# JARVIS-MoCap/JARVIS-HybridNet

Measured on AMD Instinct MI355X. Metric: multi-view frames/s (12cam 1280x1024, 23kpt, 64^3 grid), higher is better.
Workload: dtype f32; 1 GPU; BASELINE configs[2]: HybridNet 12-camera 1280x1024, 23 kpts, 64^3 grid, small/small; cameras=12, joints=23, grid=64, streams=3, parallelism=single GPU, 3 time batches in flight on 3 HIP streams, hipgraph=False

## Files before the change

include/jarvis_hip.h:

```cpp
#ifndef JARVIS_HIP_H
#define JARVIS_HIP_H
#include <stdint.h>

#ifdef __cplusplus
extern "C" {
#endif

#define JH_ABI_VERSION 4

const char* jh_last_error(void);
int jh_abi_version(void);

#define JH_PRECISION_DEFAULT (-1)
#define JH_PRECISION_F32 0
#define JH_PRECISION_BF16X3 1
#define JH_PRECISION_BF16X3_WIDE 2
int jh_set_precision(int mode);
int jh_get_precision(void);

typedef struct jh_params jh_params;
int jh_params_create(jh_params** out);
int jh_params_set(jh_params* p, const char* key, const float* host, int64_t numel);
void jh_params_destroy(jh_params* p);

// ... 222 lines not shown
  const float *se_wr_host, *se_br_host, *se_we_host, *se_be_host;
  const double* se_pool_host;
} jh_op_operand;
int jh_op_conv_operand(int nd, int kind, int k, int stride, int pad, int cin, int cout,
                       const float* w_host, const float* b_host, const float* x_dev, int n, int d, int h,
                       int w, const float* gate_dev, const jh_op_operand* operand, float* y_dev, void* stream);
int jh_op_se_gate(const double* pool_host, int n, int c, int squeeze, float inv_hw, const float* wr_host,
                  const float* br_host, const float* we_host, const float* be_host, float* gate_dev, void* stream);
int jh_op_norm_apply(const float* x_dev, int n, int c, int d, int h, int w, const double* sums_host, int act,
                     const float* r1_dev, const double* r1_sums_host, const float* r2_dev, int write_y, int want_pool,
                     int min_block_kb, float* y_dev, double* pool_host, void* stream);
int jh_op_depthwise(int k, int c, const float* w_host, const float* x_dev, int n, int h, int w,
                    int norm_act, float* y_dev, void* stream);
int jh_op_depthwise_pool(int k, int c, const float* w_host, const float* x_dev, int n, int h, int w,
                         float* y_dev, float* pool_dev, void* stream);

int jh_op_yuv420_to_bgr(const uint8_t* frames_dev, int format, int n, int h, int w, uint8_t* out_bgr_dev,
                        void* stream);
int jh_op_yuv_surface_to_bgr(const uint8_t* frames_dev, const jh_yuv_surface* surface, int n, int h, int w,
                             uint8_t* out_bgr_dev, void* stream);
int jh_op_sensor_to_bgr(const uint8_t* frames_dev, const jh_sensor_surface* surface, int n, int h, int w,
                        uint8_t* out_bgr_dev, void* stream);

int64_t jh_joint_argmax_all_workspace_bytes(int n, int hh, int wh, int jp);
int jh_op_joint_argmax_all(const float* heat_dev, int n, int hh, int wh, int j, int jp, int32_t* idx_dev,
                           float* max_dev, void* workspace_dev, int64_t workspace_bytes, void* stream);

int jh_op_bifpn_node(int n_in, const int* modes, const float* weights, int act, int n, int c, int cout,
                     int h, int w, const float* x0_dev, const float* x1_dev, const float* x2_dev,
                     const float* dw_host, const float* pw_host, const float* bias_host, float* y_dev,
// ... 7 lines not shown
```

jarvis-hybridnet_amd/_native.py:

```python
import ctypes
import math
import os
from typing import NamedTuple

import torch

_HERE = os.path.dirname(os.path.abspath(__file__))
LIB_PATH = os.environ.get("JH_LIBRARY_PATH") or os.path.join(_HERE, "libjarvis_hip.so")
_lib = None

c_void_p, c_int, c_float, c_int64 = ctypes.c_void_p, ctypes.c_int, ctypes.c_float, ctypes.c_int64
c_char_p = ctypes.c_char_p


class PredictorConfig(ctypes.Structure):
    _fields_ = [("num_cameras", ctypes.c_int32), ("num_joints", ctypes.c_int32),
                ("center_size", ctypes.c_int32), ("bbox", ctypes.c_int32),
                ("roi_cube_size", c_float), ("grid_spacing", c_float),
                ("center_model", ctypes.c_int32), ("kp_model", ctypes.c_int32),
                ("img_h", ctypes.c_int32), ("img_w", ctypes.c_int32),
                ("time_batch", ctypes.c_int32), ("time_batch_3d", ctypes.c_int32),
                ("cam_lo", ctypes.c_int32),
                ("cam_n", ctypes.c_int32), ("mean", c_float * 3), ("std", c_float * 3),
                ("precision", ctypes.c_int32)]
# ... 159 lines not shown
    "jh_predictor_debug": (c_int, [c_void_p, c_void_p, c_void_p, c_void_p, c_void_p, c_void_p]),
    "jh_predictor_hybridnet_forward": (c_int, [c_void_p] * 9),
    "jh_op_conv": (c_int, [c_int] * 7 + [c_void_p, c_void_p, c_void_p] + [c_int] * 4 +
                   [c_void_p, c_int, c_void_p, c_void_p]),
    "jh_deconv4_window_launches": (ctypes.c_long, []),
    "jh_conv_form": (c_int, [c_int] * 12 + [c_char_p, c_int]),
    "jh_op_conv_operand": (c_int, [c_int] * 7 + [c_void_p, c_void_p, c_void_p] + [c_int] * 4 +
                           [c_void_p, ctypes.POINTER(OpOperand), c_void_p, c_void_p]),
    "jh_op_se_gate": (c_int, [c_void_p, c_int, c_int, c_int, c_float] + [c_void_p] * 6),
    "jh_op_norm_apply": (c_int, [c_void_p] + [c_int] * 5 + [c_void_p, c_int, c_void_p, c_void_p, c_void_p, c_int,
                                                           c_int, c_int, c_void_p, c_void_p, c_void_p]),
    "jh_op_depthwise": (c_int, [c_int, c_int, c_void_p, c_void_p, c_int, c_int, c_int, c_int,
                                c_void_p, c_void_p]),
    "jh_op_depthwise_pool": (c_int, [c_int, c_int, c_void_p, c_void_p, c_int, c_int, c_int, c_void_p, c_void_p,
                                     c_void_p]),
    "jh_op_yuv420_to_bgr": (c_int, [c_void_p, c_int, c_int, c_int, c_int, c_void_p, c_void_p]),
    "jh_op_bifpn_node": (c_int, [c_int, ctypes.POINTER(c_int), ctypes.POINTER(c_float), c_int, c_int, c_int,
                                 c_int, c_int, c_int, c_void_p, c_void_p, c_void_p, c_void_p, c_void_p,
                                 c_void_p, c_void_p, c_void_p]),
}


def symbols():
    return sorted(_SIGS)


def lib():
    global _lib
    if _lib is None:
        if not os.path.isfile(LIB_PATH):
# ... 332 lines not shown
```

jarvis-hybridnet_amd/csrc/api.hip:

```cpp
#include <cstring>
#include <memory>
#include "../../include/jarvis_hip.h"
#include <cstdlib>
#include "nets.h"
#include "bifpn_node.h"
#include "views2d.h"
#include "subjects.h"

namespace jh {
static thread_local std::string g_err;
void set_error(const std::string& msg) { g_err = msg; }
}

using namespace jh;

struct jh_params { ParamMap map; };
struct jh_efftrack { EffTrackPlan plan; };
struct jh_v2v { V2VPlan plan; };

namespace {

struct Scratch {
  std::vector<void*> ptrs;
  ~Scratch() { for (void* p : ptrs) (void)hipFree(p); }
// ... 1554 lines not shown
  if (sc.get(reinterpret_cast<void**>(&stats), nst * sizeof(double))) return 1;
  if (sc.get(reinterpret_cast<void**>(&pool), npl * sizeof(double))) return 1;
  JH_CHECK_HIP(hipMemsetAsync(stats, 0, nst * sizeof(double), s));
  JH_CHECK_HIP(hipMemsetAsync(pool, 0, npl * sizeof(double), s));
  if (launch_to_channel_last(x_dev, x, s)) return 1;
  if (launch_depthwise(x, wd, k, y.p, stats, s, pool)) return 1;
  if (launch_from_channel_last(y, y_dev, s)) return 1;
  std::vector<double> hp(npl);
  JH_CHECK_HIP(hipMemcpyAsync(hp.data(), pool, npl * sizeof(double), hipMemcpyDeviceToHost, s));
  JH_CHECK_HIP(hipStreamSynchronize(s));
  std::vector<float> out((size_t)n * c);
  for (int i = 0; i < n; ++i)
    for (int ch = 0; ch < c; ++ch) {
      const double* q = hp.data() + ((size_t)i * x.Cp + ch) * kLimbs;
      out[(size_t)i * c + ch] = (float)((q[0] + q[1]) + q[2]);
    }
  JH_CHECK_HIP(hipMemcpy(pool_dev, out.data(), out.size() * sizeof(float), hipMemcpyHostToDevice));
  return 0;
}

static size_t carve_joint_argmax_all(Carver& c, int n, int hh, int wh, int jp, float** pmax, int** pidx) {
  const size_t k = joint_argmax_all_partials(n, hh, wh, jp);
  *pmax = c.take<float>(k);
  *pidx = c.take<int>(k);
  return c.off;
}

int64_t jh_joint_argmax_all_workspace_bytes(int n, int hh, int wh, int jp) {
  if (n < 1 || hh < 1 || wh < 1 || jp < 8 || jp % 8 || jp > 256) return 0;
  Carver c(nullptr, 0);
// ... 88 lines not shown
```

jarvis-hybridnet_amd/csrc/conv_pw_direct.hip:

```cpp
#include "conv_mfma.h"

namespace jh {

namespace {
typedef float pf4 __attribute__((ext_vector_type(4)));
typedef unsigned pu4 __attribute__((ext_vector_type(4)));

template <int KW, int NCB, int MRU>
__global__ __launch_bounds__(256) void conv_pw_direct_kernel(const ConvArgs a, int rb_per_wave) {
  __shared__ float nrm_s[4][2][64];
  const int lane = threadIdx.x & 63;
  const int wave = __builtin_amdgcn_readfirstlane(threadIdx.x >> 6);
  const int px = lane & 15, kq = lane >> 4;
  const int n = blockIdx.y;
  const int P = a.Hin * a.Win;
  const int nrb = P >> 4;
  const int rb0 = (blockIdx.x * 4 + wave) * rb_per_wave;
  const int rb1 = min(nrb, rb0 + rb_per_wave);
  if (rb0 >= nrb) return;

  float aw[KW][4][NCB];
#pragma unroll
  for (int u = 0; u < KW; ++u)
#pragma unroll
    for (int i = 0; i < 4; ++i) {
      const int c = 16 * u + 4 * kq + i;
#pragma unroll
      for (int cb = 0; cb < NCB; ++cb) {
        const int idx = (((c >> 3) * NCB + cb) * 64 + ((c & 7) >> 1) * 16 + px) * 2 + (c & 1);
        aw[u][i][cb] = c < a.cin_p ? a.w[idx] : 0.f;
      }
    }
  const bool normed = a.in_stats != nullptr;
  pf4 mu4[KW], rs4[KW], g4[KW];
#pragma unroll
  for (int u = 0; u < KW; ++u) { mu4[u] = (pf4){0.f, 0.f, 0.f, 0.f}; rs4[u] = (pf4){1.f, 1.f, 1.f, 1.f}; g4[u] = rs4[u]; }
  if (normed) {
    float m = 0.f, r = 1.f;
    if (lane < a.cin_p) {
      const double* st = a.in_stats + ((size_t)n * a.cin_p + lane) * kStatW;
      const double mu = exact_read(st) * (double)a.in_inv;
      double var = exact_read(st + kLimbs) * (double)a.in_inv - mu * mu;
      if (var < 0.0) var = 0.0;
      m = (float)mu;
      r = (float)(1.0 / sqrt(var + 1e-5));
    }
    nrm_s[wave][0][lane] = m;
    nrm_s[wave][1][lane] = r;
    __builtin_amdgcn_wave_barrier();
#pragma unroll
    for (int u = 0; u < KW; ++u)
      if (16 * u + 4 * kq < a.cin_p) {
        mu4[u] = *reinterpret_cast<const pf4*>(&nrm_s[wave][0][16 * u + 4 * kq]);
        rs4[u] = *reinterpret_cast<const pf4*>(&nrm_s[wave][1][16 * u + 4 * kq]);
      }
  }
  const bool gated = a.gate != nullptr || a.se.pool != nullptr;
  if (a.gate) {
#pragma unroll
    for (int u = 0; u < KW; ++u)
      if (16 * u + 4 * kq < a.cin_p) g4[u] = *reinterpret_cast<const pf4*>(a.gate + (size_t)n * a.cin_p + 16 * u + 4 * kq);
// ... 46 lines not shown

  pf4 t1[NCB], t2[NCB], pv[NCB];
#pragma unroll
  for (int cb = 0; cb < NCB; ++cb) { t1[cb] = (pf4){0.f, 0.f, 0.f, 0.f}; t2[cb] = t1[cb]; pv[cb] = t1[cb]; }
  bool first = true;

  auto load = [&](int rb, pf4 (&x)[KW]) __attribute__((always_inline)) {
#pragma unroll
    for (int u = 0; u < KW; ++u)
      x[u] = __builtin_bit_cast(pf4, __builtin_amdgcn_raw_buffer_load_b128(xrs, xoff[u], rb * xrb, 0));
  };
  auto compute = [&](int rb, pf4 (&x)[KW]) __attribute__((always_inline)) {
#pragma unroll
    for (int u = 0; u < KW; ++u) {
      pf4 v = x[u];
      if (normed) {
        v = (v - mu4[u]) * rs4[u];
        if (act == ACT_SILU) {
#pragma unroll
          for (int j = 0; j < 4; ++j) v[j] = silu_fast(v[j]);
        } else if (act == ACT_RELU) {
#pragma unroll
          for (int j = 0; j < 4; ++j) v[j] = fmaxf(v[j], 0.f);
        }
      }
      if (gated) v *= g4[u];
      x[u] = v;
    }
    f32x4 acc[NCB];
#pragma unroll
    for (int cb = 0; cb < NCB; ++cb) acc[cb] = (f32x4){0.f, 0.f, 0.f, 0.f};
#pragma unroll
    for (int u = 0; u < KW; ++u)
#pragma unroll
      for (int i = 0; i < 4; ++i)
#pragma unroll
        for (int cb = 0; cb < NCB; ++cb)
          acc[cb] = __builtin_amdgcn_mfma_f32_16x16x4f32(aw[u][i][cb], x[u][i], acc[cb], 0, 0, 0);
#pragma unroll
    for (int cb = 0; cb < NCB; ++cb) {
// ... 85 lines not shown
```

jarvis-hybridnet_amd/csrc/elementwise.hip:

```cpp
#include "jh_common.h"

namespace jh {

__device__ __forceinline__ float act_apply(float v, int act) {
  if (act == ACT_RELU) return fmaxf(v, 0.f);
  if (act == ACT_SILU) return v / (1.f + expf(-v));
  return v;
}

__device__ __forceinline__ void block_channel_reduce(float4 s1, float4 s2, int nvals, int q,
                                                     int rows, int tid, bool active,
                                                     double* dst, int dst_stride, float* sm) {
  if (active) {
    const int c4 = tid % q, r = tid / q;
    float4* p = reinterpret_cast<float4*>(sm) + ((size_t)r * q + c4) * nvals;
    p[0] = s1;
    if (nvals == 2) p[1] = s2;
  }
  __syncthreads();
  for (int i = tid; i < q * 4 * nvals; i += blockDim.x) {
    const int comp = i & 3, v = (i >> 2) % nvals, c4 = (i >> 2) / nvals;
    float acc = 0.f;
    for (int r = 0; r < rows; ++r) acc += sm[(((size_t)r * q + c4) * nvals + v) * 4 + comp];
    exact_add(dst + ((size_t)(c4 * 4 + comp) * dst_stride + v) * kLimbs, (double)acc);
// ... 50 lines not shown
    __syncthreads();
  }
  const size_t base = (size_t)n * P * Cp + c4 * 4;
  const int p0 = blockIdx.x * ppb;
  const int p1 = min(P, p0 + ppb);
  float4 ps = make_float4(0, 0, 0, 0);
  auto act1 = [](float v) __attribute__((always_inline)) {
    if (ACT == ACT_RELU) return fmaxf(v, 0.f);
    if (ACT == ACT_SILU) return silu_fast(v);
    return v;
  };
  auto finish = [&](float4 v, float4 a1, float4 a2, size_t off) __attribute__((always_inline)) {
    v.x = (v.x - mean.x) * rstd.x; v.y = (v.y - mean.y) * rstd.y;
    v.z = (v.z - mean.z) * rstd.z; v.w = (v.w - mean.w) * rstd.w;
    if (R1N) {
      a1.x = fmaxf((a1.x - mean1.x) * rstd1.x, 0.f); a1.y = fmaxf((a1.y - mean1.y) * rstd1.y, 0.f);
      a1.z = fmaxf((a1.z - mean1.z) * rstd1.z, 0.f); a1.w = fmaxf((a1.w - mean1.w) * rstd1.w, 0.f);
    }
    if (R1) { v.x += a1.x; v.y += a1.y; v.z += a1.z; v.w += a1.w; }
    v.x = act1(v.x); v.y = act1(v.y); v.z = act1(v.z); v.w = act1(v.w);
    if (R2) { v.x += a2.x; v.y += a2.y; v.z += a2.z; v.w += a2.w; }
    if (Y) *reinterpret_cast<float4*>(y + off) = v;
    ps.x += v.x; ps.y += v.y; ps.z += v.z; ps.w += v.w;
  };
  if (active) {
    constexpr int UN = 4;
    int p = p0 + row;
    for (; p + (UN - 1) * rows < p1; p += UN * rows) {
      float4 v[UN], a1[UN], a2[UN];
#pragma unroll
      for (int u = 0; u < UN; ++u) {
        const size_t off = base + (size_t)(p + u * rows) * Cp;
// ... 21 lines not shown
                      int min_block_kb) {
  const int P = (int)x.pixels();
  const int q = x.Cp / 4;
  JH_REQUIRE(q >= 1 && q <= 256, "channel count out of range for norm_apply");
  int bt = 256;
  for (int cand = 512; cand <= 1024; cand *= 2)
    if ((cand / q) * q * bt > (bt / q) * q * cand + cand * bt / 16) bt = cand;
  const int rows = bt / q;
  int iters = 8;
  while ((P + rows * iters - 1) / (rows * iters) > 64 && iters < 64) iters *= 2;
  while ((long)rows * iters * x.Cp * 4 < (long)min_block_kb * 1024 && iters < 64 && rows * iters < P) iters *= 2;
  const int ppb = rows * iters;
  dim3 grid((P + ppb - 1) / ppb, x.N);
  const size_t sm = ((pool ? (size_t)rows * q * 4 : 0) + (stats ? (size_t)2 * x.Cp : 0)) * sizeof(float);
  if (r1_stats) {
    JH_REQUIRE(stats && r1 && y && act == ACT_RELU && !pool, "norm_apply: normalised residual operand");
    if (r2)
      hipLaunchKernelGGL((norm_apply_kernel<ACT_RELU, true, true, true, true>), grid, dim3(bt), sm, s, x.p, stats, eps,
                         r1, r2, y, pool, P, x.Cp, ppb, r1_stats);
    else
      hipLaunchKernelGGL((norm_apply_kernel<ACT_RELU, true, false, true, true>), grid, dim3(bt), sm, s, x.p, stats, eps,
                         r1, r2, y, pool, P, x.Cp, ppb, r1_stats);
    JH_CHECK_HIP(hipGetLastError());
    return 0;
  }
#define JH_NA(A, B1, B2, BY)                                                                              \
  if (act == A && (r1 != nullptr) == B1 && (r2 != nullptr) == B2 && (y != nullptr) == BY) {             \
    hipLaunchKernelGGL((norm_apply_kernel<A, B1, B2, BY>), grid, dim3(bt), sm, s, x.p, stats, eps, r1, r2, y, \
                       pool, P, x.Cp, ppb, nullptr);                                                               \
    JH_CHECK_HIP(hipGetLastError());                                                                      \
    return 0;                                                                                             \
  }
// ... 30 lines not shown
      g = 1.f / (1.f + expf(-acc));
    }
    gate[(size_t)n * Cp + c] = g;
  }
}

int launch_se_gate(const double* pool, int N, int C, int Cp, int S, float inv_hw, const float* wr,
                   const float* br, const float* we, const float* be, float* gate,
                   hipStream_t s) {
  hipLaunchKernelGGL(se_gate_kernel, dim3(N), dim3(256), (C + S) * sizeof(float), s, pool, C, Cp,
                     S, inv_hw, wr, br, we, be, gate);
  JH_CHECK_HIP(hipGetLastError());
  return 0;
}

template <int K, int CC, bool POOL = false, int TT = 16>
__global__ __launch_bounds__(256) void depthwise_lds_kernel(
    const float* __restrict__ x, const float* __restrict__ w, float* __restrict__ y,
    double* __restrict__ stats, int H, int W, int Cp, double* __restrict__ pool = nullptr) {
  constexpr int T = TT, HT = T + K - 1, SP = CC + 4;
  static_assert(T % 4 == 0, "tiles are made of 4-pixel strips");
  constexpr int QN = CC / 4, SL = 256 / QN;
  constexpr int QS = QN == 8 ? 3 : 2;
  static_assert(CC == 32 || CC == 16, "channel chunk");
  extern __shared__ __attribute__((aligned(16))) float sm[];
  float* wl = sm + HT * HT * SP;
  const int tid = threadIdx.x;
  const int tiles_x = (W + T - 1) / T;
  const BlockId bid = xcd_block();
  const int ox0 = (bid.x % tiles_x) * T, oy0 = (bid.x / tiles_x) * T;
  const int c0 = bid.y * CC;
  const int n = bid.z;
  const int q = min(CC, Cp - c0) >> 2;
  typedef float df2 __attribute__((ext_vector_type(2)));
  typedef float df4 __attribute__((ext_vector_type(4)));
  const int lc4 = tid & (QN - 1), slot = tid >> QS;
  df4 wv = (df4){0.f, 0.f, 0.f, 0.f};
  if (tid < K * K * QN && lc4 < q)
    wv = *reinterpret_cast<const df4*>(w + (size_t)(tid >> QS) * Cp + c0 + lc4 * 4);
  const __amdgpu_buffer_rsrc_t rs = __builtin_amdgcn_make_buffer_rsrc(
      const_cast<float*>(x + (size_t)n * H * W * Cp), 0, (int)((size_t)H * W * Cp * 4), 0x00020000);
  constexpr int NPX = HT * HT, ITERS = (NPX + SL - 1) / SL;
  df4 v[ITERS];
#pragma unroll
  for (int u = 0; u < ITERS; ++u) {
    const int pix = u * SL + slot;
    const int px = pix % HT, py = pix / HT;
    const int iy = oy0 + py - K / 2, ix = ox0 + px - K / 2;
    const bool ok = pix < NPX && lc4 < q && iy >= 0 && iy < H && ix >= 0 && ix < W;
    const int off = ok ? ((iy * W + ix) * Cp + c0 + lc4 * 4) * 4 : (int)0x80000000;
    v[u] = __builtin_bit_cast(df4, __builtin_amdgcn_raw_buffer_load_b128(rs, off, 0, 0));
  }
  if (tid < K * K * QN) *reinterpret_cast<df4*>(wl + (tid >> QS) * CC + lc4 * 4) = wv;
#pragma unroll
  for (int u = 0; u < ITERS; ++u) {
    const int pix = u * SL + slot;
    if (pix < NPX) *reinterpret_cast<df4*>(sm + pix * SP + lc4 * 4) = v[u];
  }
  const int c4 = tid & (QN - 1);
  const bool active = c4 < q;
  __syncthreads();
  df2 s1l = (df2){0.f, 0.f}, s1h = s1l, s2l = s1l, s2h = s1l, pvl = s1l, pvh = s1l;
  int cnt = 0;
  constexpr int SPR = T / 4, NSTR = T * SPR, NJ = (NSTR + SL - 1) / SL, NK = POOL ? NJ : 1, UNR = POOL ? NJ : 1;
  static_assert(!POOL || NJ <= 2, "registers for the strips of a thread");
  df2 alk[NK][4], ahk[NK][4];
  unsigned okmk[NK];
#pragma unroll
  for (int jj = 0; jj < NK; ++jj) okmk[jj] = 0;
  if (active) {
#pragma unroll UNR
    for (int j = 0; j < NJ; ++j) {
// ... 59 lines not shown
    for (int i = tid; i < q * 8 * 8; i += 256) {
      const int part = i & 7, val = i >> 3;
      const int comp = val & 3, sq = (val >> 2) & 1, cq = val >> 3;
      double acc = 0.0;
#pragma unroll
      for (int r = 0; r < SL / 8; ++r) acc += smd[(((size_t)(part * (SL / 8) + r) * QN + cq) * 2 + sq) * 4 + comp];
      red2[val * 8 + part] = acc;
    }
    __syncthreads();
    double* tot = red2 + QN * 8 * 8;
    for (int i = tid; i < q * 8; i += 256) {
      const int comp = i & 3, sq = (i >> 2) & 1, cq = i >> 3;
      double acc = 0.0;
#pragma unroll
      for (int r = 0; r < 8; ++r) acc += red2[i * 8 + r];
      exact_add_rounded(stats + (((size_t)n * Cp + c0 + cq * 4 + comp) * 2 + sq) * kLimbs, acc);
      if (POOL) tot[i] = acc;
    }
    if (POOL) {
      float* mr = reinterpret_cast<float*>(tot + QN * 8);
      float* red2f = reinterpret_cast<float*>(red2);
      __syncthreads();
      if (tid < q * 4) {
        const int cq = tid >> 2, comp = tid & 3;
        const double P = (double)(H * W);
        const double mu = tot[(cq * 2 + 0) * 4 + comp] / P;
        double var = tot[(cq * 2 + 1) * 4 + comp] / P - mu * mu;
        if (var < 0.0) var = 0.0;
        mr[tid] = (float)mu;
        mr[CC + tid] = (float)(1.0 / sqrt(var + 1e-5));
      }
      __syncthreads();
// ... 23 lines not shown
        red2f[val * 8 + part] = acc;
      }
      __syncthreads();
      for (int i = tid; i < q * 4; i += 256) {
        float acc = 0.f;
#pragma unroll
        for (int r = 0; r < 8; ++r) acc += red2f[i * 8 + r];
        exact_add(pool + ((size_t)n * Cp + c0 + i) * kLimbs, (double)acc);
      }
    }
  }
}

bool depthwise_can_pool(int H, int W) {
  return H <= 20 && W <= 20;
}

int launch_depthwise(const Act& x, const float* w, int k, float* y, double* stats, hipStream_t s, double* pool) {
  JH_REQUIRE(x.D == 1, "depthwise is 2D only");
  JH_REQUIRE(k == 3 || k == 5, "depthwise kernel size must be 3 or 5");
  const int tt = (std::max(x.H, x.W) > 16 && std::max(x.H, x.W) <= 20) ? 20 : 16;
  const int tiles = ((x.H + tt - 1) / tt) * ((x.W + tt - 1) / tt);
  if (pool) {
    JH_REQUIRE(depthwise_can_pool(x.H, x.W) && tiles == 1 && stats,
               "fused depthwise pooled sums need a one-tile image and statistics");
    dim3 grid(1, (x.Cp + 15) / 16, x.N);
    const int ht = tt + k - 1;
    size_t lds = (size_t)(ht * ht * (16 + 4) + k * k * 16) * sizeof(float);
    const size_t red = (size_t)(64 * 4 * 8 + 4 * 8 * 8 + 4 * 8) * sizeof(double) + 2 * 16 * sizeof(float);
    if (lds < red) lds = red;
// ... 159 lines not shown
```

jarvis-hybridnet_amd/csrc/jh_common.h:

```cpp
#pragma once
#include <hip/hip_runtime.h>
#include <cstdlib>
#include <cstdint>
#include <cstdio>
#include <cstring>
#include <string>
#include <vector>

namespace jh {

constexpr int kWave = 64;

#define JH_ENV_KNOB(name) ([]() -> int { static const int v = [] { const char* e = getenv(name); return e ? atoi(e) : -1; }(); return v; }())

inline int round_up(int v, int m) { return (v + m - 1) / m * m; }
inline int cpad(int c) { return round_up(c, 8); }

void set_error(const std::string& msg);
#define JH_CHECK_HIP(expr)                                                     \
  do {                                                                         \
    hipError_t _e = (expr);                                                    \
    if (_e != hipSuccess) {                                                    \
      jh::set_error(std::string(#expr) + ": " + hipGetErrorString(_e));        \
      return 1;                                                                \
// ... 141 lines not shown

ConvDesc conv_desc(int nd, int k, int stride, int pad, int cin, int cout);
ConvDesc deconv2d_k4s2p1_desc(int cin, int cout);
ConvDesc deconv3d_k2s2_desc(int cin, int cout);
long deconv4_window_launches();

int launch_norm_apply(const Act& x, const double* stats, double eps, int act,
                      const float* r1, const float* r2, float* y, double* pool,
                      hipStream_t s, const double* r1_stats = nullptr, int min_block_kb = 0);
int launch_se_gate(const double* pool, int N, int C, int Cp, int S, float inv_hw,
                   const float* wr, const float* br, const float* we, const float* be,
                   float* gate, hipStream_t s);
bool depthwise_can_pool(int H, int W);
int launch_depthwise(const Act& x, const float* w, int k, float* y, double* stats,
                     hipStream_t s, double* pool = nullptr);
enum FuseMode { FUSE_SAME = 0, FUSE_UP2 = 1, FUSE_UP4 = 2, FUSE_POOL2 = 3 };
struct FuseArgs {
  const float* in[3];
  int mode[3];
  float w[3];
  int n_in;
  int act;
};
int launch_fuse(const FuseArgs& f, const Act& out, hipStream_t s);
int launch_maxpool2(const Act& x, float* y, hipStream_t s);

struct BlockId { unsigned x, y, z; };

constexpr int kLimbs = 3;
constexpr int kStatW = 2 * kLimbs;
#if defined(__HIPCC__)
__device__ __forceinline__ void exact_add(double* dst, double p) {
  const double h = rint(p * 0x1p-16) * 0x1p16;
  const double r = p - h;
  const double m = rint(r * 0x1p20) * 0x1p-20;
  const double l = rint((r - m) * 0x1p56) * 0x1p-56;
  if (h != 0.0) unsafeAtomicAdd(dst + 0, h);
  if (m != 0.0) unsafeAtomicAdd(dst + 1, m);
  if (l != 0.0) unsafeAtomicAdd(dst + 2, l);
}
__device__ __forceinline__ double exact_read(const double* src) { return (src[0] + src[1]) + src[2]; }
__device__ __forceinline__ void stat_add(double* st, float s1, float s2) {
  exact_add(st, (double)s1);
  exact_add(st + kLimbs, (double)s2);
}
__device__ __forceinline__ void exact_add_rounded(double* dst, double p) {
  const double a = fabs(p);
  double q;
  int slot;
  if (a < 0x1p5) { q = rint(p * 0x1p35) * 0x1p-35; slot = 2; }
  else if (a < 0x1p15) { q = rint(p * 0x1p25) * 0x1p-25; slot = 1; }
  else { q = rint(p * 0x1p15) * 0x1p-15; slot = 0; }
  if (q != 0.0) unsafeAtomicAdd(dst + slot, q);
}
__device__ __forceinline__ void stat_add(double* st, double s1, double s2) {
  exact_add_rounded(st, s1);
  exact_add_rounded(st + kLimbs, s2);
}
__device__ __forceinline__ void stat_acc(double& s1, double& s2, float v) {
  const double d = (double)v;
  s1 += d;
  s2 = fma(d, d, s2);
}
#endif

#if defined(__HIPCC__)
__device__ __forceinline__ unsigned xcd_linear(unsigned L, unsigned total) {
  const unsigned q = total >> 3, r = total & 7u, x = L & 7u, s = L >> 3;
// ... 99 lines not shown
```

jarvis-hybridnet_amd/csrc/nets.hip:

```cpp
#include <cmath>
#include <cstring>
#include <cstdlib>
#include "nets.h"
#include "bifpn_node.h"

namespace jh {

Profiler& profiler() {
  static Profiler p;
  return p;
}
void Profiler::begin(const std::string& name, double flops, double bytes, hipStream_t s) {
  ProfRec r{name, flops, bytes, nullptr, nullptr, 0.f};
  (void)hipEventCreate(&r.e0);
  (void)hipEventCreate(&r.e1);
  (void)hipEventRecord(r.e0, s);
  recs.push_back(r);
}
void Profiler::end(hipStream_t s) { (void)hipEventRecord(recs.back().e1, s); }
int Profiler::finish() {
  JH_CHECK_HIP(hipDeviceSynchronize());
  for (auto& r : recs) {
    if (!r.e0) continue;
    JH_CHECK_HIP(hipEventElapsedTime(&r.ms, r.e0, r.e1));
// ... 157 lines not shown
  float r[3], sum = 0.f;
  for (int i = 0; i < n; ++i) { r[i] = p[i] > 0.f ? p[i] : 0.f; sum += r[i]; }
  for (int i = 0; i < n; ++i) w[i] = r[i] / (sum + 1e-4f);
}
}

void EffTrackPlan::materialise(Ref* x) {
  if (x->st < 0) return;
  add_norm(x->a, (size_t)x->st, x->act, nullptr, nullptr, x->a.p, -1);
  x->st = -1;
}

int EffTrackPlan::mbconv(const ParamMap& pm, const std::string& p, int stage, int k, int stride,
                         int cin, int cout, int expand, Ref* xin, Ref* outr) {
  const bool skip = (stride == 1 && cin == cout);
  if (skip || (stage >= 4 && expand == 1)) materialise(xin);
  const Ref xr = *xin;
  const Act& x = xr.a;
  Act* out = &outr->a;
  const int mid = cin * expand;
  const int squeeze = std::max(1, (int)(cin * 0.25));
  const int Ho = (x.H + 2 * (k / 2) - k) / stride + 1, Wo = (x.W + 2 * (k / 2) - k) / stride + 1;
  Act raw;
  if (new_act(x.N, 1, Ho, Wo, mid, &raw)) return 1;
  size_t st1 = 0;
  const size_t pool = scratch((size_t)raw.N * raw.Cp * kLimbs);
  bool pooled = false;
  if (stage < 4) {
    if (add_conv(pm, conv_desc(2, k, stride, k / 2, cin, mid), p + "_depthwise_conv.weight", "",
                 false, x, raw, nullptr, true, &st1, xr.st, xr.inv, xr.act)) return 1;
  } else {
    Act e = x;
    if (expand != 1) {
      if (new_act(x.N, 1, x.H, x.W, mid, &e)) return 1;
      if (add_conv(pm, conv_desc(2, 1, 1, 0, cin, mid), p + "_expand_conv.weight", "", false, x, e,
                   nullptr, false, nullptr, xr.st, xr.inv, xr.act)) return 1;
    }
    JH_REQUIRE(stride == 1, "depthwise stages are stride 1");
    const float* w = nullptr;
    if (get(pm, p + "_depthwise_conv.weight", (size_t)mid * k * k, &w)) return 1;
    float* wd = nullptr;
    if (upload(taps_major(w, mid, k * k, raw.Cp), &wd)) return 1;
    st1 = scratch((size_t)raw.N * raw.Cp * kStatW);
    pooled = depthwise_can_pool(Ho, Wo);
    push(std::string("depthwise_k") + std::to_string(k) + (pooled ? "pool" : ""), 2.0 * raw.N * raw.pixels() * mid * k * k,
         8.0 * raw.N * raw.pixels() * mid, [this, e, wd, k, raw, st1, pool, pooled](hipStream_t s) {
      return launch_depthwise(e, wd, k, raw.p, sc(st1), s, pooled ? sc(pool) : nullptr);
    });
  }
  if (!pooled) add_norm(raw, st1, ACT_SILU, nullptr, nullptr, nullptr, (long)pool);
  const float *wr, *br, *we, *be;
  if (get(pm, p + "_se_reduce.weight", (size_t)squeeze * mid, &wr)) return 1;
  if (get(pm, p + "_se_reduce.bias", squeeze, &br)) return 1;
  if (get(pm, p + "_se_expand.weight", (size_t)mid * squeeze, &we)) return 1;
  if (get(pm, p + "_se_expand.bias", mid, &be)) return 1;
  float *dwr, *dbr, *dwe, *dbe, *gate = nullptr;
  if (upload(std::vector<float>(wr, wr + (size_t)squeeze * mid), &dwr)) return 1;
  if (upload(std::vector<float>(br, br + squeeze), &dbr)) return 1;
  if (upload(std::vector<float>(we, we + (size_t)mid * squeeze), &dwe)) return 1;
  if (upload(std::vector<float>(be, be + mid), &dbe)) return 1;
  const float inv_hw = 1.f / (float)(Ho * Wo);
  const bool se_fused = raw.N <= 32;
  SeGate seg;
  seg.wr = dwr; seg.br = dbr; seg.we = dwe; seg.be = dbe; seg.C = mid; seg.S = squeeze; seg.inv_hw = inv_hw;
  if (!se_fused) {
    if (alloc(reinterpret_cast<void**>(&gate), (size_t)raw.N * raw.Cp * sizeof(float))) return 1;
    push("se_gate", 4.0 * raw.N * mid * squeeze, 8.0 * raw.N * mid,
         [this, pool, raw, mid, squeeze, inv_hw, dwr, dbr, dwe, dbe, gate](hipStream_t s) {
      return launch_se_gate(sc(pool), raw.N, mid, raw.Cp, squeeze, inv_hw, dwr, dbr, dwe, dbe, gate, s);
    });
  }
  if (new_act(x.N, 1, Ho, Wo, cout, out)) return 1;
  size_t st2 = 0;
  if (add_conv(pm, conv_desc(2, 1, 1, 0, mid, cout), p + "_project_conv.weight", "", false, raw,
               *out, gate, true, &st2, (long)st1, 1.f / (float)(Ho * Wo), ACT_SILU,
               se_fused ? &seg : nullptr, se_fused ? (long)pool : -1)) return 1;
  if (skip) {
    add_norm(*out, st2, ACT_NONE, x.p, nullptr, out->p, -1);
    outr->st = -1;
  } else {
    outr->st = (long)st2;
    outr->inv = 1.f / (float)(Ho * Wo);
    outr->act = ACT_NONE;
  }
  return 0;
}

int EffTrackPlan::lateral(const ParamMap& pm, const std::string& p, int cout, const Ref& xr,
                          Ref* out) {
  const Act& x = xr.a;
  if (new_act(x.N, 1, x.H, x.W, cout, &out->a)) return 1;
  size_t st = 0;
  if (add_conv(pm, conv_desc(2, 1, 1, 0, x.C, cout), p + ".0.weight", p + ".0.bias", false, x,
// ... 292 lines not shown
```

Baseline: 2171 multi-view frames/s.

## Fuse MBConv expand pointwise conv into one-tile pooled depthwise kernel

For small late-stage MBConv blocks whose image fits in one depthwise tile, the expand 1x1 conv now runs with MFMA inside the depthwise kernel. The input is normalised on the fly and the expanded activation goes straight into the LDS halo tile, so the expanded tensor is never written to and reread from global memory and one launch per block is dropped. Skip connections can also consume the raw, un-normalised input through a normalised-residual norm_apply path instead of materialising it first. In exchange the expand GEMM is repeated for each 16-channel block with no reuse across blocks, and it needs more LDS.

```diff
diff --git a/include/jarvis_hip.h b/include/jarvis_hip.h
--- a/include/jarvis_hip.h
+++ b/include/jarvis_hip.h
@@ -260,6 +260,9 @@
                     int norm_act, float* y_dev, void* stream);
 int jh_op_depthwise_pool(int k, int c, const float* w_host, const float* x_dev, int n, int h, int w,
                          float* y_dev, float* pool_dev, void* stream);
+int jh_op_expand_depthwise_pool(int k, int cin, int mid, const float* we_host, const float* wd_host, const float* x_dev,
+                                int n, int h, int w, const double* in_sums_host, int in_act, float* y_dev,
+                                float* pool_dev, void* stream);
 
 int jh_op_yuv420_to_bgr(const uint8_t* frames_dev, int format, int n, int h, int w, uint8_t* out_bgr_dev,
                         void* stream);
diff --git a/jarvis-hybridnet_amd/_native.py b/jarvis-hybridnet_amd/_native.py
--- a/jarvis-hybridnet_amd/_native.py
+++ b/jarvis-hybridnet_amd/_native.py
@@ -197,6 +197,8 @@
                                 c_void_p, c_void_p]),
     "jh_op_depthwise_pool": (c_int, [c_int, c_int, c_void_p, c_void_p, c_int, c_int, c_int, c_void_p, c_void_p,
                                      c_void_p]),
+    "jh_op_expand_depthwise_pool": (c_int, [c_int, c_int, c_int, c_void_p, c_void_p, c_void_p, c_int, c_int, c_int,
+                                            c_void_p, c_int, c_void_p, c_void_p, c_void_p]),
     "jh_op_yuv420_to_bgr": (c_int, [c_void_p, c_int, c_int, c_int, c_int, c_void_p, c_void_p]),
     "jh_op_bifpn_node": (c_int, [c_int, ctypes.POINTER(c_int), ctypes.POINTER(c_float), c_int, c_int, c_int,
                                  c_int, c_int, c_int, c_void_p, c_void_p, c_void_p, c_void_p, c_void_p,
diff --git a/jarvis-hybridnet_amd/csrc/api.hip b/jarvis-hybridnet_amd/csrc/api.hip
--- a/jarvis-hybridnet_amd/csrc/api.hip
+++ b/jarvis-hybridnet_amd/csrc/api.hip
@@ -1592,6 +1592,50 @@
     for (int ch = 0; ch < c; ++ch) {
       const double* q = hp.data() + ((size_t)i * x.Cp + ch) * kLimbs;
       out[(size_t)i * c + ch] = (float)((q[0] + q[1]) + q[2]);
+    }
+  JH_CHECK_HIP(hipMemcpy(pool_dev, out.data(), out.size() * sizeof(float), hipMemcpyHostToDevice));
+  return 0;
+}
+
+int jh_op_expand_depthwise_pool(int k, int cin, int mid, const float* we_host, const float* wd_host, const float* x_dev,
+                                int n, int h, int w, const double* in_sums_host, int in_act, float* y_dev,
+                                float* pool_dev, void* stream) {
+  hipStream_t s = static_cast<hipStream_t>(stream);
+  JH_REQUIRE(we_host && wd_host && x_dev && y_dev && pool_dev && n >= 1 && cin >= 1 && mid >= 1, "bad argument");
+  JH_REQUIRE(in_act >= ACT_NONE && in_act <= ACT_SILU, "jh_op_expand_depthwise_pool: in_act");
+  JH_REQUIRE(depthwise_can_pool(h, w), "jh_op_expand_depthwise_pool: the image must be one tile");
+  Scratch sc;
+  Act x, y;
+  if (sc.act(n, 1, h, w, cin, &x)) return 1;
+  if (sc.act(n, 1, h, w, mid, &y)) return 1;
+  const std::vector<float> wt = taps_major(wd_host, mid, k * k, y.Cp);
+  float* wd; double *stats = nullptr, *pool = nullptr;
+  if (op_upload(sc, wt.data(), wt.size(), &wd)) return 1;
+  ConvWeights ew;
+  if (pack_conv_weights(conv_desc(2, 1, 1, 0, cin, mid), we_host, nullptr, false, WeightLayout::Plain, &ew)) return 1;
+  struct FreeW { ConvWeights* w; ~FreeW() { free_conv_weights(w); } } free_ew{&ew};
+  InNorm in;
+  if (in_sums_host) {
+    double* st = nullptr;
+    if (op_upload_stats(sc, in_sums_host, n, cin, x.Cp, &st)) return 1;
+    in.stats = st; in.inv = 1.f / (float)x.pixels(); in.act = in_act;
+  }
+  const size_t nst = (size_t)n * y.Cp * kStatW, npl = (size_t)n * y.Cp * kLimbs;
+  if (sc.get(reinterpret_cast<void**>(&stats), nst * sizeof(double))) return 1;
+  if (sc.get(reinterpret_cast<void**>(&pool), npl * sizeof(double))) return 1;
+  JH_CHECK_HIP(hipMemsetAsync(stats, 0, nst * sizeof(double), s));
+  JH_CHECK_HIP(hipMemsetAsync(pool, 0, npl * sizeof(double), s));
+  if (launch_to_channel_last(x_dev, x, s)) return 1;
+  if (launch_expand_depthwise(x, ew, in, wd, k, y, stats, pool, s)) return 1;
+  if (launch_from_channel_last(y, y_dev, s)) return 1;
+  std::vector<double> hp(npl);
+  JH_CHECK_HIP(hipMemcpyAsync(hp.data(), pool, npl * sizeof(double), hipMemcpyDeviceToHost, s));
+  JH_CHECK_HIP(hipStreamSynchronize(s));
+  std::vector<float> out((size_t)n * mid);
+  for (int i = 0; i < n; ++i)
+    for (int ch = 0; ch < mid; ++ch) {
+      const double* q = hp.data() + ((size_t)i * y.Cp + ch) * kLimbs;
+      out[(size_t)i * mid + ch] = (float)((q[0] + q[1]) + q[2]);
     }
   JH_CHECK_HIP(hipMemcpy(pool_dev, out.data(), out.size() * sizeof(float), hipMemcpyHostToDevice));
   return 0;
diff --git a/jarvis-hybridnet_amd/csrc/conv_pw_direct.hip b/jarvis-hybridnet_amd/csrc/conv_pw_direct.hip
--- a/jarvis-hybridnet_amd/csrc/conv_pw_direct.hip
+++ b/jarvis-hybridnet_amd/csrc/conv_pw_direct.hip
@@ -1,10 +1,9 @@
 #include "conv_mfma.h"
+#include "pw_operand.h"
 
 namespace jh {
 
 namespace {
-typedef float pf4 __attribute__((ext_vector_type(4)));
-typedef unsigned pu4 __attribute__((ext_vector_type(4)));
 
 template <int KW, int NCB, int MRU>
 __global__ __launch_bounds__(256) void conv_pw_direct_kernel(const ConvArgs a, int rb_per_wave) {
@@ -27,8 +26,7 @@
       const int c = 16 * u + 4 * kq + i;
 #pragma unroll
       for (int cb = 0; cb < NCB; ++cb) {
-        const int idx = (((c >> 3) * NCB + cb) * 64 + ((c & 7) >> 1) * 16 + px) * 2 + (c & 1);
-        aw[u][i][cb] = c < a.cin_p ? a.w[idx] : 0.f;
+        aw[u][i][cb] = c < a.cin_p ? a.w[pw_weight_index(c, NCB, cb, px)] : 0.f;
       }
     }
   const bool normed = a.in_stats != nullptr;
@@ -37,14 +35,7 @@
   for (int u = 0; u < KW; ++u) { mu4[u] = (pf4){0.f, 0.f, 0.f, 0.f}; rs4[u] = (pf4){1.f, 1.f, 1.f, 1.f}; g4[u] = rs4[u]; }
   if (normed) {
     float m = 0.f, r = 1.f;
-    if (lane < a.cin_p) {
-      const double* st = a.in_stats + ((size_t)n * a.cin_p + lane) * kStatW;
-      const double mu = exact_read(st) * (double)a.in_inv;
-      double var = exact_read(st + kLimbs) * (double)a.in_inv - mu * mu;
-      if (var < 0.0) var = 0.0;
-      m = (float)mu;
-      r = (float)(1.0 / sqrt(var + 1e-5));
-    }
+    if (lane < a.cin_p) pw_in_norm(a.in_stats + ((size_t)n * a.cin_p + lane) * kStatW, a.in_inv, &m, &r);
     nrm_s[wave][0][lane] = m;
     nrm_s[wave][1][lane] = r;
     __builtin_amdgcn_wave_barrier();
@@ -121,16 +112,7 @@
 #pragma unroll
     for (int u = 0; u < KW; ++u) {
       pf4 v = x[u];
-      if (normed) {
-        v = (v - mu4[u]) * rs4[u];
-        if (act == ACT_SILU) {
-#pragma unroll
-          for (int j = 0; j < 4; ++j) v[j] = silu_fast(v[j]);
-        } else if (act == ACT_RELU) {
-#pragma unroll
-          for (int j = 0; j < 4; ++j) v[j] = fmaxf(v[j], 0.f);
-        }
-      }
+      if (normed) v = pw_in_apply(v, mu4[u], rs4[u], act);
       if (gated) v *= g4[u];
       x[u] = v;
     }
diff --git a/jarvis-hybridnet_amd/csrc/elementwise.hip b/jarvis-hybridnet_amd/csrc/elementwise.hip
--- a/jarvis-hybridnet_amd/csrc/elementwise.hip
+++ b/jarvis-hybridnet_amd/csrc/elementwise.hip
@@ -1,4 +1,5 @@
 #include "jh_common.h"
+#include "pw_operand.h"
 
 namespace jh {
 
@@ -88,8 +89,9 @@
     v.x = (v.x - mean.x) * rstd.x; v.y = (v.y - mean.y) * rstd.y;
     v.z = (v.z - mean.z) * rstd.z; v.w = (v.w - mean.w) * rstd.w;
     if (R1N) {
-      a1.x = fmaxf((a1.x - mean1.x) * rstd1.x, 0.f); a1.y = fmaxf((a1.y - mean1.y) * rstd1.y, 0.f);
-      a1.z = fmaxf((a1.z - mean1.z) * rstd1.z, 0.f); a1.w = fmaxf((a1.w - mean1.w) * rstd1.w, 0.f);
+      a1.x = (a1.x - mean1.x) * rstd1.x; a1.y = (a1.y - mean1.y) * rstd1.y;
+      a1.z = (a1.z - mean1.z) * rstd1.z; a1.w = (a1.w - mean1.w) * rstd1.w;
+      if (ACT == ACT_RELU) { a1.x = fmaxf(a1.x, 0.f); a1.y = fmaxf(a1.y, 0.f); a1.z = fmaxf(a1.z, 0.f); a1.w = fmaxf(a1.w, 0.f); }
     }
     if (R1) { v.x += a1.x; v.y += a1.y; v.z += a1.z; v.w += a1.w; }
     v.x = act1(v.x); v.y = act1(v.y); v.z = act1(v.z); v.w = act1(v.w);
@@ -141,8 +143,11 @@
   dim3 grid((P + ppb - 1) / ppb, x.N);
   const size_t sm = ((pool ? (size_t)rows * q * 4 : 0) + (stats ? (size_t)2 * x.Cp : 0)) * sizeof(float);
   if (r1_stats) {
-    JH_REQUIRE(stats && r1 && y && act == ACT_RELU && !pool, "norm_apply: normalised residual operand");
-    if (r2)
+    JH_REQUIRE(stats && r1 && y && (act == ACT_RELU || (act == ACT_NONE && !r2)) && !pool, "norm_apply: normalised residual operand");
+    if (act == ACT_NONE)
+      hipLaunchKernelGGL((norm_apply_kernel<ACT_NONE, true, false, true, true>), grid, dim3(bt), sm, s, x.p, stats, eps,
+                         r1, r2, y, pool, P, x.Cp, ppb, r1_stats);
+    else if (r2)
       hipLaunchKernelGGL((norm_apply_kernel<ACT_RELU, true, true, true, true>), grid, dim3(bt), sm, s, x.p, stats, eps,
                          r1, r2, y, pool, P, x.Cp, ppb, r1_stats);
     else
@@ -203,10 +208,18 @@
   return 0;
 }
 
-template <int K, int CC, bool POOL = false, int TT = 16>
+struct DwExpand {
+  const float* x = nullptr;
+  const float* w = nullptr;
+  int cin_p = 0, ncb = 0;
+  const double* in_stats = nullptr;
+  float in_inv = 0.f;
+  int in_act = 0;
+};
+template <int K, int CC, bool POOL = false, int TT = 16, bool EXPAND = false>
 __global__ __launch_bounds__(256) void depthwise_lds_kernel(
     const float* __restrict__ x, const float* __restrict__ w, float* __restrict__ y,
-    double* __restrict__ stats, int H, int W, int Cp, double* __restrict__ pool = nullptr) {
+    double* __restrict__ stats, int H, int W, int Cp, double* __restrict__ pool = nullptr, const DwExpand ex = DwExpand()) {
   constexpr int T = TT, HT = T + K - 1, SP = CC + 4;
   static_assert(T % 4 == 0, "tiles are made of 4-pixel strips");
   constexpr int QN = CC / 4, SL = 256 / QN;
@@ -227,24 +240,93 @@
   df4 wv = (df4){0.f, 0.f, 0.f, 0.f};
   if (tid < K * K * QN && lc4 < q)
     wv = *reinterpret_cast<const df4*>(w + (size_t)(tid >> QS) * Cp + c0 + lc4 * 4);
-  const __amdgpu_buffer_rsrc_t rs = __builtin_amdgcn_make_buffer_rsrc(
-      const_cast<float*>(x + (size_t)n * H * W * Cp), 0, (int)((size_t)H * W * Cp * 4), 0x00020000);
-  constexpr int NPX = HT * HT, ITERS = (NPX + SL - 1) / SL;
-  df4 v[ITERS];
-#pragma unroll
-  for (int u = 0; u < ITERS; ++u) {
-    const int pix = u * SL + slot;
-    const int px = pix % HT, py = pix / HT;
-    const int iy = oy0 + py - K / 2, ix = ox0 + px - K / 2;
-    const bool ok = pix < NPX && lc4 < q && iy >= 0 && iy < H && ix >= 0 && ix < W;
-    const int off = ok ? ((iy * W + ix) * Cp + c0 + lc4 * 4) * 4 : (int)0x80000000;
-    v[u] = __builtin_bit_cast(df4, __builtin_amdgcn_raw_buffer_load_b128(rs, off, 0, 0));
-  }
-  if (tid < K * K * QN) *reinterpret_cast<df4*>(wl + (tid >> QS) * CC + lc4 * 4) = wv;
-#pragma unroll
-  for (int u = 0; u < ITERS; ++u) {
-    const int pix = u * SL + slot;
-    if (pix < NPX) *reinterpret_cast<df4*>(sm + pix * SP + lc4 * 4) = v[u];
+  static_assert(!EXPAND || (POOL && CC == 16), "the expand stage belongs to the one-tile pooled form");
+  if constexpr (EXPAND) {
+    const int P = H * W, cin_p = ex.cin_p;
+    float* nrm = wl + K * K * CC;
+    const bool normed = ex.in_stats != nullptr;
+    if (normed)
+      for (int c = tid; c < cin_p; c += 256)
+        pw_in_norm(ex.in_stats + ((size_t)n * cin_p + c) * kStatW, ex.in_inv, nrm + c, nrm + cin_p + c);
+    for (int pix = tid; pix < HT * HT; pix += 256) {
+      const int iy = pix / HT - K / 2, ix = pix % HT - K / 2;
+      if (iy < 0 || iy >= H || ix < 0 || ix >= W) {
+#pragma unroll
+        for (int j = 0; j < CC / 4; ++j) *reinterpret_cast<df4*>(sm + pix * SP + j * 4) = (df4){0.f, 0.f, 0.f, 0.f};
+      }
+    }
+    if (tid < K * K * QN) *reinterpret_cast<df4*>(wl + (tid >> QS) * CC + lc4 * 4) = wv;
+    if (normed) __syncthreads();
+    const int lane = tid & 63, wave = tid >> 6, px = lane & 15, kq = lane >> 4;
+    const int cb = c0 / CC;
+    constexpr int NRB = ((T * T + 15) / 16 + 3) / 4;
+    const __amdgpu_buffer_rsrc_t xrs = __builtin_amdgcn_make_buffer_rsrc(
+        const_cast<float*>(ex.x + (size_t)n * P * cin_p), 0, (int)((size_t)P * cin_p * 4), 0x00020000);
+    df4 acc[NRB];
+#pragma unroll
+    for (int m = 0; m < NRB; ++m) acc[m] = (df4){0.f, 0.f, 0.f, 0.f};
+    const int kw = (cin_p + 15) >> 4;
+    for (int u0 = 0; u0 < kw; u0 += 2) {
+      pf4 xv[2][NRB];
+      float aw[2][4];
+#pragma unroll
+      for (int uu = 0; uu < 2; ++uu) {
+        const int cw = 16 * (u0 + uu) + 4 * kq;
+        const bool okc = cw < cin_p;
+#pragma unroll
+        for (int i = 0; i < 4; i += 2) {
+          const float2 w2 = okc ? *reinterpret_cast<const float2*>(ex.w + pw_weight_index(cw + i, ex.ncb, cb, px))
+                                : make_float2(0.f, 0.f);
+          aw[uu][i] = w2.x; aw[uu][i + 1] = w2.y;
+        }
+#pragma unroll
+        for (int m = 0; m < NRB; ++m) {
+          const int p = (wave + 4 * m) * 16 + px;
+          const int off = (okc && p < P) ? (p * cin_p + cw) * 4 : (int)0x80000000;
+          xv[uu][m] = __builtin_bit_cast(pf4, __builtin_amdgcn_raw_buffer_load_b128(xrs, off, 0, 0));
+        }
+      }
+#pragma unroll
+      for (int uu = 0; uu < 2; ++uu) {
+        const int cw = 16 * (u0 + uu) + 4 * kq;
+        if (u0 + uu >= kw) break;
+        if (normed && cw < cin_p) {
+          const pf4 mu = *reinterpret_cast<const pf4*>(nrm + cw), rs = *reinterpret_cast<const pf4*>(nrm + cin_p + cw);
+#pragma unroll
+          for (int m = 0; m < NRB; ++m) xv[uu][m] = pw_in_apply(xv[uu][m], mu, rs, ex.in_act);
+        }
+#pragma unroll
+        for (int i = 0; i < 4; ++i)
+#pragma unroll
+          for (int m = 0; m < NRB; ++m)
+            acc[m] = __builtin_amdgcn_mfma_f32_16x16x4f32(aw[uu][i], xv[uu][m][i], acc[m], 0, 0, 0);
+      }
+    }
+#pragma unroll
+    for (int m = 0; m < NRB; ++m) {
+      const int p = (wave + 4 * m) * 16 + px;
+      if (p < P) *reinterpret_cast<df4*>(sm + ((p / W + K / 2) * HT + p % W + K / 2) * SP + kq * 4) = acc[m];
+    }
+  } else {
+    const __amdgpu_buffer_rsrc_t rs = __builtin_amdgcn_make_buffer_rsrc(
+        const_cast<float*>(x + (size_t)n * H * W * Cp), 0, (int)((size_t)H * W * Cp * 4), 0x00020000);
+    constexpr int NPX = HT * HT, ITERS = (NPX + SL - 1) / SL;
+    df4 v[ITERS];
+#pragma unroll
+    for (int u = 0; u < ITERS; ++u) {
+      const int pix = u * SL + slot;
+      const int px = pix % HT, py = pix / HT;
+      const int iy = oy0 + py - K / 2, ix = ox0 + px - K / 2;
+      const bool ok = pix < NPX && lc4 < q && iy >= 0 && iy < H && ix >= 0 && ix < W;
+      const int off = ok ? ((iy * W + ix) * Cp + c0 + lc4 * 4) * 4 : (int)0x80000000;
+      v[u] = __builtin_bit_cast(df4, __builtin_amdgcn_raw_buffer_load_b128(rs, off, 0, 0));
+    }
+    if (tid < K * K * QN) *reinterpret_cast<df4*>(wl + (tid >> QS) * CC + lc4 * 4) = wv;
+#pragma unroll
+    for (int u = 0; u < ITERS; ++u) {
+      const int pix = u * SL + slot;
+      if (pix < NPX) *reinterpret_cast<df4*>(sm + pix * SP + lc4 * 4) = v[u];
+    }
   }
   const int c4 = tid & (QN - 1);
   const bool active = c4 < q;
@@ -334,8 +416,8 @@
       double acc = 0.0;
 #pragma unroll
       for (int r = 0; r < 8; ++r) acc += red2[i * 8 + r];
-      exact_add_rounded(stats + (((size_t)n * Cp + c0 + cq * 4 + comp) * 2 + sq) * kLimbs, acc);
-      if (POOL) tot[i] = acc;
+      const double added = exact_add_rounded(stats + (((size_t)n * Cp + c0 + cq * 4 + comp) * 2 + sq) * kLimbs, acc);
+      if (POOL) tot[i] = added;
     }
     if (POOL) {
       float* mr = reinterpret_cast<float*>(tot + QN * 8);
@@ -389,6 +471,31 @@
 
 bool depthwise_can_pool(int H, int W) {
   return H <= 20 && W <= 20;
+}
+
+int launch_expand_depthwise(const Act& x, const ConvWeights& ew, const InNorm& in, const float* w, int k, const Act& y,
+                            double* stats, double* pool, hipStream_t s) {
+  JH_REQUIRE(x.D == 1 && y.D == 1 && x.N == y.N && x.H == y.H && x.W == y.W, "expand + depthwise: one image size");
+  JH_REQUIRE(k == 3 || k == 5, "depthwise kernel size must be 3 or 5");
+  JH_REQUIRE(depthwise_can_pool(y.H, y.W) && stats && pool, "expand + depthwise needs a one-tile image, statistics and pooled sums");
+  JH_REQUIRE(ew.layout == WeightLayout::Plain && ew.cin_p == x.Cp && ew.cout_p16 == round_up(y.Cp, 16) && !ew.bias,
+             "expand weights: Plain layout of a bias-free cin -> mid pointwise layer");
+  JH_REQUIRE(x.Cp % 8 == 0 && x.Cp <= 256, "expand + depthwise: input channels");
+  const int tt = std::max(y.H, y.W) > 16 ? 20 : 16;
+  DwExpand ex;
+  ex.x = x.p; ex.w = ew.w; ex.cin_p = x.Cp; ex.ncb = ew.cout_p16 / 16;
+  ex.in_stats = in.stats; ex.in_inv = in.inv; ex.in_act = in.act;
+  dim3 grid(1, (y.Cp + 15) / 16, y.N);
+  const int ht = tt + k - 1;
+  size_t lds = (size_t)(ht * ht * (16 + 4) + k * k * 16 + 2 * x.Cp) * sizeof(float);
+  const size_t red = (size_t)(64 * 4 * 8 + 4 * 8 * 8 + 4 * 8) * sizeof(double) + 2 * 16 * sizeof(float);
+  if (lds < red) lds = red;
+#define JH_DWX(K, TTV) hipLaunchKernelGGL((depthwise_lds_kernel<K, 16, true, TTV, true>), grid, dim3(256), lds, s, (const float*)nullptr, w, y.p, stats, y.H, y.W, y.Cp, pool, ex)
+  if (k == 3) { if (tt == 20) JH_DWX(3, 20); else JH_DWX(3, 16); }
+  else { if (tt == 20) JH_DWX(5, 20); else JH_DWX(5, 16); }
+#undef JH_DWX
+  JH_CHECK_HIP(hipGetLastError());
+  return 0;
 }
 
 int launch_depthwise(const Act& x, const float* w, int k, float* y, double* stats, hipStream_t s, double* pool) {
diff --git a/jarvis-hybridnet_amd/csrc/jh_common.h b/jarvis-hybridnet_amd/csrc/jh_common.h
--- a/jarvis-hybridnet_amd/csrc/jh_common.h
+++ b/jarvis-hybridnet_amd/csrc/jh_common.h
@@ -179,6 +179,8 @@
 bool depthwise_can_pool(int H, int W);
 int launch_depthwise(const Act& x, const float* w, int k, float* y, double* stats,
                      hipStream_t s, double* pool = nullptr);
+int launch_expand_depthwise(const Act& x, const ConvWeights& ew, const InNorm& in, const float* w, int k, const Act& y,
+                            double* stats, double* pool, hipStream_t s);
 enum FuseMode { FUSE_SAME = 0, FUSE_UP2 = 1, FUSE_UP4 = 2, FUSE_POOL2 = 3 };
 struct FuseArgs {
   const float* in[3];
@@ -209,7 +211,7 @@
   exact_add(st, (double)s1);
   exact_add(st + kLimbs, (double)s2);
 }
-__device__ __forceinline__ void exact_add_rounded(double* dst, double p) {
+__device__ __forceinline__ double exact_add_rounded(double* dst, double p) {
   const double a = fabs(p);
   double q;
   int slot;
@@ -217,6 +219,7 @@
   else if (a < 0x1p15) { q = rint(p * 0x1p25) * 0x1p-25; slot = 1; }
   else { q = rint(p * 0x1p15) * 0x1p-15; slot = 0; }
   if (q != 0.0) unsafeAtomicAdd(dst + slot, q);
+  return q;
 }
 __device__ __forceinline__ void stat_add(double* st, double s1, double s2) {
   exact_add_rounded(st, s1);
diff --git a/jarvis-hybridnet_amd/csrc/nets.hip b/jarvis-hybridnet_amd/csrc/nets.hip
--- a/jarvis-hybridnet_amd/csrc/nets.hip
+++ b/jarvis-hybridnet_amd/csrc/nets.hip
@@ -195,13 +195,17 @@
 int EffTrackPlan::mbconv(const ParamMap& pm, const std::string& p, int stage, int k, int stride,
                          int cin, int cout, int expand, Ref* xin, Ref* outr) {
   const bool skip = (stride == 1 && cin == cout);
-  if (skip || (stage >= 4 && expand == 1)) materialise(xin);
+  const int Ho = (xin->a.H + 2 * (k / 2) - k) / stride + 1, Wo = (xin->a.W + 2 * (k / 2) - k) / stride + 1;
+  const char* mk = getenv("JH_MBCONV16");
+  const bool one_tile = !(mk && atoi(mk) == 0) && depthwise_can_pool(Ho, Wo);
+  const bool expand_fused = one_tile && stage >= 4 && expand != 1;
+  const bool raw_skip = one_tile && skip && xin->act == ACT_NONE && (stage < 4 || expand_fused);
+  if (!raw_skip && (skip || (stage >= 4 && expand == 1))) materialise(xin);
   const Ref xr = *xin;
   const Act& x = xr.a;
   Act* out = &outr->a;
   const int mid = cin * expand;
   const int squeeze = std::max(1, (int)(cin * 0.25));
-  const int Ho = (x.H + 2 * (k / 2) - k) / stride + 1, Wo = (x.W + 2 * (k / 2) - k) / stride + 1;
   Act raw;
   if (new_act(x.N, 1, Ho, Wo, mid, &raw)) return 1;
   size_t st1 = 0;
@@ -212,7 +216,14 @@
                  false, x, raw, nullptr, true, &st1, xr.st, xr.inv, xr.act)) return 1;
   } else {
     Act e = x;
-    if (expand != 1) {
+    ConvWeights ew;
+    if (expand_fused) {
+      const float* wh = nullptr;
+      if (get(pm, p + "_expand_conv.weight", (size_t)cin * mid, &wh)) return 1;
+      if (pack_conv_weights(conv_desc(2, 1, 1, 0, cin, mid), wh, nullptr, false, WeightLayout::Plain, &ew)) return 1;
+      convs_.push_back(ew);
+      bytes_ += (size_t)ew.cin_p * ew.cout_p16 * sizeof(float);
+    } else if (expand != 1) {
       if (new_act(x.N, 1, x.H, x.W, mid, &e)) return 1;
       if (add_conv(pm, conv_desc(2, 1, 1, 0, cin, mid), p + "_expand_conv.weight", "", false, x, e,
                    nullptr, false, nullptr, xr.st, xr.inv, xr.act)) return 1;
@@ -224,10 +235,24 @@
     if (upload(taps_major(w, mid, k * k, raw.Cp), &wd)) return 1;
     st1 = scratch((size_t)raw.N * raw.Cp * kStatW);
     pooled = depthwise_can_pool(Ho, Wo);
-    push(std::string("depthwise_k") + std::to_string(k) + (pooled ? "pool" : ""), 2.0 * raw.N * raw.pixels() * mid * k * k,
-         8.0 * raw.N * raw.pixels() * mid, [this, e, wd, k, raw, st1, pool, pooled](hipStream_t s) {
-      return launch_depthwise(e, wd, k, raw.p, sc(st1), s, pooled ? sc(pool) : nullptr);
-    });
+    if (expand_fused) {
+      const double px = (double)raw.N * raw.pixels();
+      const long xst = xr.st;
+      const float xinv = xr.inv;
+      const int xact = xr.act;
+      push("depthwise_k" + std::to_string(k) + "pool_x" + std::to_string(cin), 2.0 * px * mid * (k * k + cin),
+           4.0 * (px * (cin + mid) + (double)mid * (cin + k * k)),
+           [this, x, ew, xst, xinv, xact, wd, k, raw, st1, pool](hipStream_t s) {
+        InNorm in;
+        if (xst >= 0) { in.stats = sc((size_t)xst); in.inv = xinv; in.act = xact; }
+        return launch_expand_depthwise(x, ew, in, wd, k, raw, sc(st1), sc(pool), s);
+      });
+    } else {
+      push(std::string("depthwise_k") + std::to_string(k) + (pooled ? "pool" : ""), 2.0 * raw.N * raw.pixels() * mid * k * k,
+           8.0 * raw.N * raw.pixels() * mid, [this, e, wd, k, raw, st1, pool, pooled](hipStream_t s) {
+        return launch_depthwise(e, wd, k, raw.p, sc(st1), s, pooled ? sc(pool) : nullptr);
+      });
+    }
   }
   if (!pooled) add_norm(raw, st1, ACT_SILU, nullptr, nullptr, nullptr, (long)pool);
   const float *wr, *br, *we, *be;
@@ -257,7 +282,7 @@
                *out, gate, true, &st2, (long)st1, 1.f / (float)(Ho * Wo), ACT_SILU,
                se_fused ? &seg : nullptr, se_fused ? (long)pool : -1)) return 1;
   if (skip) {
-    add_norm(*out, st2, ACT_NONE, x.p, nullptr, out->p, -1);
+    add_norm(*out, st2, ACT_NONE, x.p, nullptr, out->p, -1, raw_skip ? xr.st : -1);
     outr->st = -1;
   } else {
     outr->st = (long)st2;
diff --git a/jarvis-hybridnet_amd/csrc/pw_operand.h b/jarvis-hybridnet_amd/csrc/pw_operand.h
--- /dev/null
+++ b/jarvis-hybridnet_amd/csrc/pw_operand.h
@@ -0,0 +1,35 @@
+#pragma once
+#include "jh_common.h"
+
+namespace jh {
+
+#if defined(__HIPCC__)
+typedef float pf4 __attribute__((ext_vector_type(4)));
+typedef unsigned pu4 __attribute__((ext_vector_type(4)));
+
+__device__ __forceinline__ int pw_weight_index(int c, int ncb, int cb, int px) {
+  return (((c >> 3) * ncb + cb) * 64 + ((c & 7) >> 1) * 16 + px) * 2 + (c & 1);
+}
+
+__device__ __forceinline__ void pw_in_norm(const double* st, float inv, float* m, float* r) {
+  const double mu = exact_read(st) * (double)inv;
+  double var = exact_read(st + kLimbs) * (double)inv - mu * mu;
+  if (var < 0.0) var = 0.0;
+  *m = (float)mu;
+  *r = (float)(1.0 / sqrt(var + 1e-5));
+}
+
+__device__ __forceinline__ pf4 pw_in_apply(pf4 v, pf4 mu, pf4 rs, int act) {
+  v = (v - mu) * rs;
+  if (act == ACT_SILU) {
+#pragma unroll
+    for (int j = 0; j < 4; ++j) v[j] = silu_fast(v[j]);
+  } else if (act == ACT_RELU) {
+#pragma unroll
+    for (int j = 0; j < 4; ++j) v[j] = fmaxf(v[j], 0.f);
+  }
+  return v;
+}
+#endif
+
+}
```

After: 2176 multi-view frames/s (median of 3 runs). About the same (+0.2%).
